# TinyMPC/TinyMPC

Hardware: AMD Instinct MI355X
Metric: QP solves/sec (+ ADMM iters/sec), 64k-batch quadrotor hover (higher is better)
Workload: dtype f64; 1 GPU; quadrotor_hovering (nx=12, nu=4, N=10), 65536 identical instances per GPU, closed-loop MPC steps from a cold start (BASELINE configs[1]); batch_per_gpu=65536, total_batch=65536, parallelism=batch-sharded x1, mpc_steps_per_launch=8, stats_exchange=none (one rank), launcher=plain process

## Files before the change

### tinympc_amd/csrc/admm_kernel.hip.h

```cpp
#pragma once
#include <hip/hip_runtime.h>
#include <stdint.h>

namespace tinympc_amd {

enum : int {
    VEC_CB = 0,
    VEC_CF = 1,
    VEC_QR = 2,
    VEC_SMASK = 3,
    VEC_NIM = 4,
    VEC_SOCFLAG = 5,
    VEC_CONE_BASE = 6,
    VEC_CONE_MU = 7,
    VEC_RHO = 8,
    VEC_LINFLAG = 9,
    VEC_TLINFLAG = 10,
    VEC_COUNT = 16,
};
struct LaneTab {
    int cols, lw;
    constexpr int MB() const { return 0; }
    constexpr int MF1() const { return cols * lw; }
    constexpr int MF2() const { return 2 * cols * lw; }
// ... 361 lines not shown
            DPP_REP(TINYMPC_FUSED_NX, HFWD_COL_A_HI)
            "v_mov_b64 %[xn], %[t]\n\t"
            "v_add_f64 %[gnew], %[tt], -%[vn]\n\t"
            DPP_REP(TINYMPC_FUSED_NU, HFWD_COL_B_LO)
            "s_nop 0\n\t"
            DPP_REP(TINYMPC_FUSED_NU, HFWD_COL_B_HI)
            : [tt] "=&v"(tt), [vm] "=&v"(vm), [vn] "=&v"(vn), [xn] "=&v"(xn), [t] "+&v"(t), [gnew] "=&v"(gnew)
            : [xi] "v"(xi), [g] "v"(g), [lo] "v"(lo), [hi] "v"(hi), FUSED_ROW_OPERANDS);
    }
#endif
}

__device__ __forceinline__ double vmax64(double a, double b) {
    double r;
    asm("v_max_f64 %0, %1, %2" : "=v"(r) : "v"(a), "v"(b));
    return r;
}
__device__ __forceinline__ double vmin64(double a, double b) {
    double r;
    asm("v_min_f64 %0, %1, %2" : "=v"(r) : "v"(a), "v"(b));
    return r;
}
__device__ __forceinline__ double pinned_sub64(double a, double b) {
    double r = a - b;
    asm volatile("" : "+v"(r));
    return r;
}
__device__ __forceinline__ double vclamp64(double lo, double hi, double t) {
    double r;
    asm("v_max_f64 %0, %1, %2\n\tv_min_f64 %0, %3, %0" : "=&v"(r) : "v"(lo), "v"(t), "v"(hi));
    return r;
}

__device__ __forceinline__ double vmax_abs64(double a, double b) {
    double r;
    asm("v_max_f64 %0, %1, |%2|" : "=v"(r) : "v"(a), "v"(b));
    return r;
}
template <bool OPAQUE>
__device__ __forceinline__ double resid_max(double a, double b) {
    if constexpr (OPAQUE) return vmax_abs64(a, b);
    else return fmax(a, fabs(b));
}

#ifndef TINYMPC_PRIM_STORE
#define TINYMPC_PRIM_STORE 1
#endif
#ifndef TINYMPC_REF_LOAD
#define TINYMPC_REF_LOAD 1
#endif
#ifndef TINYMPC_FULL_LINE_STORES
#define TINYMPC_FULL_LINE_STORES 2
#endif
__device__ __forceinline__ double load_ref(const double* p) {
#if TINYMPC_REF_LOAD == 1
    return __builtin_nontemporal_load(p);
#else
    return *p;
#endif
}
__device__ __forceinline__ void store_primal(double* p, double v) {
#if TINYMPC_PRIM_STORE == 1
    __builtin_nontemporal_store(v, p);
#elif TINYMPC_PRIM_STORE == 2
    asm volatile("global_store_dwordx2 %0, %1, off sc1" : : "v"(p), "v"(v) : "memory");
#elif TINYMPC_PRIM_STORE == 3
// ... 792 lines not shown
#pragma unroll
                        for (int s = 0; s < N; ++s) {
                            const double vc0 = soc_lane ? X[s] : 0.0;
                            sC[cw + s * SLOT_D] = vc0 - sC[cw + s * SLOT_D + PL_GC];
                            sC[cw + s * SLOT_D + PL_VC] = vc0;
                        }
                    }
                }
                if constexpr (LS) {
                    if (step > 0) {
#pragma unroll
                        for (int s = 0; s < N; ++s) { if constexpr (LSP) sLV[cl + s * CSL] = lin_lane ? X[s] : 0.0; else VL[s] = lin_lane ? X[s] : 0.0; }
                    } else if (is_state && lin_lane && !resumed) { if constexpr (LSP) sLV[cl] = x0v; else VL[0] = x0v; }
                }
                if constexpr (LT) {
                    if (step > 0) {
#pragma unroll
                        for (int s = 0; s < N; ++s) { if constexpr (LTP) sTV[cl + s * CSL] = tlin_lane ? X[s] : 0.0; else VT[s] = tlin_lane ? X[s] : 0.0; }
                    } else if (is_state && tlin_lane && !resumed) { if constexpr (LTP) sTV[cl] = x0v; else VT[0] = x0v; }
                }
                if constexpr (LPL) __builtin_amdgcn_fence(__ATOMIC_RELEASE, "wavefront");
                const int iter0 = iter_first;
                iter = iter0; solved = 0;
                if (resumed && P.check_termination > 0) checked = 1;
                int countdown = P.check_termination;
                double wr[SOC ? SPR : 1];
                bool gcz[SOC_PASSES];
#pragma unroll
                for (int p = 0; p < SOC_PASSES; ++p) gcz[p] = false;
                if constexpr (SOC) {
#pragma unroll
                    for (int d = 1; d <= SPR && d <= N; ++d) wr[(N - d) % SPR] = sC[cw + (N - d) * SLOT_D];
                }
                for (int it = iter0; it < P.max_iter; ++it) {
                    double lvr[LSP ? SPR : 1], lgr[LSP ? SPR : 1], tvr[LTP ? SPR : 1], tgr[LTP ? SPR : 1];
                    if constexpr (LPL) {
#pragma unroll
                        for (int d = 1; d <= SPR && d <= N; ++d) {
                            if constexpr (LSP) { lvr[(N - d) % SPR] = sLV[cl + (N - d) * CSL]; lgr[(N - d) % SPR] = sLG[cl + (N - d) * CSL]; }
                            if constexpr (LTP) { tvr[(N - d) % SPR] = sTV[cl + (N - d) * CSL]; tgr[(N - d) % SPR] = sTG[cl + (N - d) * CSL]; }
                        }
                    }
                    auto lin_w = [&](const int s_) { if constexpr (LSP) return lvr[s_ % SPR] - lgr[s_ % SPR]; else return VL[LSR ? s_ : 0] - GL[LSR ? s_ : 0]; };
                    auto tlin_w = [&](const int s_) { if constexpr (LTP) return tvr[s_ % SPR] - tgr[s_ % SPR]; else return VT[LTR ? s_ : 0] - GT[LTR ? s_ : 0]; };
                    double qhi;
                    {
                        double t = fma(-rho, VN[N - 1] - G[N - 1], QX[N - 1]);
                        if constexpr (SOC) t = fma(-rho, wr[(N - 1) % SPR], t);
                        if constexpr (LS) t = fma(-rho, lin_w(N - 1), t);
                        if constexpr (LT) t = fma(-rho, tlin_w(N - 1), t);
                        qhi = t;
                        if constexpr (DBG) {
                            double ql = fma(-rho, VN[N - 1] - G[N - 1], qx_last_plain);
                            if constexpr (SOC) ql = fma(-rho, wr[(N - 1) % SPR], ql);
                            if constexpr (LS) ql = fma(-rho, lin_w(N - 1), ql);
                            if constexpr (LT) ql = fma(-rho, tlin_w(N - 1), ql);
                            Qd[N - 1] = is_state ? ql : t;
                            Pd[N - 1] = t;
                        }
                    }
                    double pcur = qhi;
                    if constexpr (HALF) {
                        double tmpv = VN[N - 2] - G[N - 2];
#pragma unroll
                        for (int i = N - 2; i >= 0; --i) {
                            double qlo, res, dnp, tmpn;
                            constexpr int dummy = 0;
// ... 4 lines not shown
                            pcur = res;
                            qhi = qlo;
                        }
                        Dn[0] = fma(pcur, nim, cf);
                    }
#pragma unroll
                    for (int i = N - 2; i >= 0 && !HALF; --i) {
                        if constexpr (SOC) {
                            if (i >= SPD) wr[(i - SPD) % SPR] = sC[cw + (i - SPD) * SLOT_D];
                        }
                        if constexpr (LSP) { if (i >= SPD) { lvr[(i - SPD) % SPR] = sLV[cl + (i - SPD) * CSL]; lgr[(i - SPD) % SPR] = sLG[cl + (i - SPD) * CSL]; } }
                        if constexpr (LTP) { if (i >= SPD) { tvr[(i - SPD) % SPR] = sTV[cl + (i - SPD) * CSL]; tgr[(i - SPD) % SPR] = sTG[cl + (i - SPD) * CSL]; } }
                        if constexpr (SOC || LPL) __builtin_amdgcn_sched_barrier(0);
                        if constexpr (FUSED) {
                            double qlo, res;
                            if constexpr (SOC) fused_backward_step_soc<NX, NU>(qlo, res, VN[i], G[i], QX[i], wr[i % SPR], rho, smask, cb, pcur, qhi, mb, mb + NX);
                            else fused_backward_step<NX, NU>(qlo, res, VN[i], G[i], QX[i], rho, smask, cb, pcur, qhi, mb, mb + NX);
                            pcur = res;
                            Dn[i] = fma(res, nim, cf);
                            if constexpr (DBG) { Qd[i] = qlo; Pd[i] = res; Dd[i + 1] = res; }
                            qhi = qlo;
                            continue;
                        }
                        double qlo = fma(-rho, VN[i] - G[i], QX[i]);
                        if constexpr (SOC) qlo = fma(-rho, wr[i % SPR], qlo);
                        if constexpr (LS) qlo = fma(-rho, lin_w(i), qlo);
                        if constexpr (LT) qlo = fma(-rho, tlin_w(i), qlo);
                        const double res = ring_sum2<MODE, NX, NU>(fma(qlo, smask, cb), pcur, mb, qhi, mb + NX);
                        pcur = res;
                        Dn[i] = fma(res, nim, cf);
                        if constexpr (DBG) { Qd[i] = qlo; Pd[i] = res; Dd[i + 1] = res; }
                        qhi = qlo;
                    }
                    constexpr bool LAZY_RES = N <= 12;
                    constexpr bool TIGHT = FUSED && !HALF && LAZY_RES && !SOC && NX % 4 == 0;
                    double pmax = 0.0, dmax = 0.0;
                    auto slot_update = [&](const int s, const double lo, const double hi, const double gcv, const double glv, const double gtv) {
                        const double xi = X[s];
                        const double t = xi + G[s];
                        const double vn = TIGHT ? vclamp64(lo, hi, t) : vmin64(hi, vmax64(lo, t));
                        if constexpr (!LAZY_RES) {
                            pmax = resid_max<true>(pmax, xi - vn);
                            dmax = resid_max<true>(dmax, VP[s] - vn);
                        }
                        G[s] = t - vn;
                        VN[s] = vn;
                        if constexpr (SOC) {
                            sC[cw + s * SLOT_D] = fma(xi, socmask, gcv);
                        }
                        if constexpr (LSP) sLV[cl + s * CSL] = (lin_lane && (is_state || s >= 1)) ? (xi + glv) : 0.0;
                        if constexpr (LTP) sTV[cl + s * CSL] = (tlin_lane && (is_state || s >= 1)) ? (xi + gtv) : 0.0;
                        if constexpr (LSR || LTR) {
                            auto halfspaces = [&](double z, const double* tabk, const int nk) {
                                for (int k = 0; k < nk; ++k) {
                                    const double a = tabk[k * 16 + j];
                                    const double bk = tabk[KMAX * 16 + k * 16 + j];
                                    const double nn = tabk[2 * KMAX * 16 + k * 16 + j];
                                    const double prod = a * z;
                                    double cs = 0.0, ci = 0.0;
                                    ring1<0, NX>(cs, prod, ones);
                                    ring1<NX, NU>(ci, prod, ones);
                                    const double cv = is_state ? cs : ci;
                                    if (cv > bk) {
#pragma clang fp contract(off)
                                        const double pr = ((cv - bk) / nn) * a;
                                        z = z - pr;
                                    }
                                }
                                return z;
// ... 47 lines not shown
                                if constexpr (!LAZY_RES) {
                                    pmax = resid_max<true>(pmax, xi - vn);
                                    dmax = resid_max<true>(dmax, VP[i] - vn);
                                }
                                G[i] = gnew;
                                VN[i] = vn;
                                lo_c = lo_n; hi_c = hi_n;
                                continue;
                            }
                            fused_forward_step<NX, NU, TIGHT>(tt, vn, t, xn, xi, G[i], lo_c, hi_c, mf1, mf2);
                            X[i + 1] = xn;
                            if constexpr (!LAZY_RES) {
                                pmax = resid_max<true>(pmax, xi - vn);
                                dmax = resid_max<true>(dmax, VP[i] - vn);
                            }
                            if constexpr (TIGHT) {
                                __builtin_amdgcn_sched_barrier(0);
                                if (i > 0) G[i - 1] = pinned_sub64(tt_d, vn_d);
                                tt_d = tt; vn_d = vn;
                            } else G[i] = tt - vn;
                            VN[i] = vn;
                            if constexpr (SOC) sC[cw + i * SLOT_D] = fma(xi, socmask, gr[i % SPR]);
                            lo_c = lo_n; hi_c = hi_n;
                            continue;
                        }
                        const double t = ring_sum<MODE, 0, NX>(Dn[i], X[i], mf1);
                        X[i + 1] = ring_short<MODE, NX, NU>(t, t, mf2);
                        slot_update(i, lo_c, hi_c, gr[SOC ? i % SPR : 0], glr[LSP ? i % SPR : 0], gtr[LTP ? i % SPR : 0]);
                        lo_c = lo_n; hi_c = hi_n;
                    }
                    if constexpr (TIGHT && N >= 2) G[N - 2] = tt_d - vn_d;
                    (void)tt_d; (void)vn_d;
                    slot_update(N - 1, lo_c, hi_c, gr[SOC ? (N - 1) % SPR : 0], glr[LSP ? (N - 1) % SPR : 0], gtr[LTP ? (N - 1) % SPR : 0]);
                    if constexpr (LPL) {
                        __builtin_amdgcn_fence(__ATOMIC_RELEASE, "wavefront");
                        __builtin_amdgcn_wave_barrier();
                        if constexpr (LSP) {
                            if (lin_x_on) project_halfspace_columns<NX, KMAX, 16, 16>(j, grp, N, CSL, 0, 0, sLV, sLG, rLin, 0, P.n_lin);
                            if (lin_u_on) project_halfspace_columns<NU, KMAX, 16, 16>(j, grp, N, CSL, NX, 1, sLV, sLG, rLin, 0, P.n_lin);
                        }
                        if constexpr (LTP) {
                            if (tlin_x_on) project_halfspace_columns<NX, KMAX, 16, 16>(j, grp, N, CSL, 0, 0, sTV, sTG, rTLin, 3 * KMAX * 16, P.n_tlin);
                            if (tlin_u_on) project_halfspace_columns<NU, KMAX, 16, 16>(j, grp, N, CSL, NX, 1, sTV, sTG, rTLin, 3 * KMAX * 16, P.n_tlin);
                        }
                        __builtin_amdgcn_fence(__ATOMIC_RELEASE, "wavefront");
                        __builtin_amdgcn_wave_barrier();
                    }
                    bool conv = false;
                    auto termination = [&]() {
                        if (countdown > 0 && --countdown == 0) {
                            countdown = P.check_termination;
                            checked = 1;
                            constexpr int PS0 = N >= 2 ? 1 : 0, PS1 = N - 1;
                            auto lost = [&](const int s) {
                                return (int)(fabs(X[s] - VN[s]) >= P.tol_pri) | (int)(fabs(VP[s] - VN[s]) * rho >= P.tol_dua);
                            };
                            const bool maybe = ((int)!(rho > 0.0) | (int)!(lost(PS0) | lost(PS1))) != 0;
                            unsigned long long fold = __ballot(maybe);
                            fold &= fold >> 1; fold &= fold >> 2; fold &= fold >> 4;
                            if constexpr (!HALF) fold &= fold >> 8;
                            const bool any_row = (fold & (HALF ? 0x0101010101010101ull : 0x0001000100010001ull)) != 0ull;
                            const bool last_test = (P.max_iter - 1 - it) < P.check_termination;
                            if (last_test || any_row) {
                                if constexpr (LAZY_RES) {
#pragma unroll
                                    for (int s = 0; s < N; ++s) {
                                        pmax = resid_max<false>(pmax, X[s] - VN[s]);
                                        dmax = resid_max<false>(dmax, VP[s] - VN[s]);
                                    }
                                }
                                rp = pmax;
                                rd = dmax * rho;
                                const bool ok = (rp < P.tol_pri) && (rd < P.tol_dua);
                                const unsigned long long bal = __ballot(ok);
                                conv = ((bal >> (grp * RL)) & RMASK) == RMASK;
                            }
                        }
                    };
                    if constexpr (SOC) {
                        __builtin_amdgcn_fence(__ATOMIC_RELEASE, "wavefront");
                        __builtin_amdgcn_wave_barrier();
                        double n0 = sC[item_at[0]], n1 = sC[item_at[0] + 1], n2 = sC[item_at[0] + 2];
#pragma unroll
                        for (int d = 1; d <= SPR && d <= N; ++d) wr[(N - d) % SPR] = sC[cw + (N - d) * SLOT_D];
                        termination();
                        bool any_exact = false;
#pragma unroll
                        for (int p = 0; p < SOC_PASSES; ++p) {
                            if (p > 0 && p >= soc_passes) break;
                            const int at = item_at[p];
                            if (p > 0) { n0 = sC[at]; n1 = sC[at + 1]; n2 = sC[at + 2]; }
                            const double s0 = n0, s1 = n1, s2 = n2;
                            if (soc_all_inside(s0, s1, s2, item_mu[p])) {
                                sC[at + PL_VC] = s0; sC[at + PL_VC + 1] = s1; sC[at + PL_VC + 2] = s2;
                                if (!gcz[p]) {
                                    sC[at + PL_GC] = 0.0; sC[at + PL_GC + 1] = 0.0; sC[at + PL_GC + 2] = 0.0;
                                    gcz[p] = true;
                                }
                            } else {
                                double r0, r1, r2;
                                soc_project3(s0, s1, s2, item_mu[p], item_rmu[p], mu_pow2, r0, r1, r2);
                                const double g0 = s0 - r0, g1 = s1 - r1, g2 = s2 - r2;
                                sC[at + PL_VC] = r0; sC[at + PL_VC + 1] = r1; sC[at + PL_VC + 2] = r2;
                                sC[at + PL_GC] = g0; sC[at + PL_GC + 1] = g1; sC[at + PL_GC + 2] = g2;
                                sC[at] = r0 - g0; sC[at + 1] = r1 - g1; sC[at + 2] = r2 - g2;
                                gcz[p] = false;
                                any_exact = true;
                            }
                        }
                        if (it == iter0 && !proj_lane) {
#pragma unroll
                            for (int s = 0; s < N; ++s) sC[cw + s * SLOT_D + PL_GC] = 0.0;
                        }
                        __builtin_amdgcn_fence(__ATOMIC_RELEASE, "wavefront");
                        __builtin_amdgcn_wave_barrier();
                        if (any_exact) {
#pragma unroll
                            for (int d = 1; d <= SPR && d <= N; ++d) wr[(N - d) % SPR] = sC[cw + (N - d) * SLOT_D];
// ... 41 lines not shown
                            dual_res = grp_max16(dual_res); px_max = grp_max16(px_max); aty_max = grp_max16(aty_max); q_max = grp_max16(q_max);
                            const double pri_norm = fmax(ax_max, z_max);
                            const double dual_norm = fmax(fmax(px_max, aty_max), q_max);
                            const double eps = 1e-10;
                            const double normalized_pri = pri_res / (pri_norm + eps);
                            const double normalized_dual = dual_res / (dual_norm + eps);
                            const double ratio = normalized_pri / (normalized_dual + eps);
                            double new_rho = rho * sqrt(ratio);
                            if (P.aclip) new_rho = fmin(fmax(new_rho, P.arho_min), P.arho_max);
                            const double delta = new_rho - rho;
                            if (is_state) {
#pragma unroll
                                for (int k = 0; k < NU; ++k) mb[NX + k] = -taylor_step(-mb[NX + k], delta, (HA ? atab_i[ATAB_DK + k * 16 + j] : sTab[(16 + j) * AKC + k]));
#pragma unroll
                                for (int k = 0; k < NX; ++k) {
                                    const int e = grp * NX * NX + k + NX * j;
                                    sP[e] = taylor_step(sP[e], delta, (HA ? atab_i[ATAB_DP + k * 16 + j] : sTab[(32 + j) * AKC + k]));
                                }
                            } else if (is_input) {
#pragma unroll
                                for (int k = 0; k < NX; ++k) mf1[k] = -taylor_step(-mf1[k], delta, (HA ? atab_i[ATAB_DK + k * 16 + j] : sTab[(16 + j) * AKC + k]));
                            }
                            if (P.aC1 || P.aC2) {
                                if (j == 0) sDl[grp * ADAPT_LOG + ndl] = delta;
                                if (++ndl == ADAPT_LOG) { flush_c(ndl); ndl = 0; }
                            }
                            rho = new_rho;
                            __builtin_amdgcn_fence(__ATOMIC_RELEASE, "wavefront");
                            __builtin_amdgcn_wave_barrier();
                            QX[N - 1] = qx_last_plain;
                            terminal_term();
                        }
                    }
                    if constexpr (!SOC) termination();
                    if (conv) { solved = 1; break; }
#pragma unroll
                    for (int s = 0; s < N; ++s) VP[s] = VN[s];
                    vp_touched = true;
                }
                acc_iter += (unsigned)(iter - iter0);
                acc_solved += (unsigned)solved;
                if (P.iter_log && j == 0) P.iter_log[(size_t)step * P.batch + b] = solved ? iter : -iter;
                if (P.u0_log && is_input) P.u0_log[((size_t)step * P.batch + b) * NU + (j - NX)] = X[1];
                if constexpr (PE) {
                    double* const elog = late_arg<double>(__builtin_offsetof(SolveArgs, est_log));
                    if (elog && is_state) elog[((size_t)step * P.batch + b) * NX + j] = X[0];
                }
                if (nsteps > 1) {
                    x0v = is_state ? X[1] : 0.0;
                    if constexpr (PM) {
                        if (step + 1 < nsteps) {
                            const size_t cell = true_cell();
                            double xt = true_x0(step, cell);
                            [[maybe_unused]] double est_next = 0.0;
                            if constexpr (PE) est_next = (iter > iter0) ? predicted(X[0], X[1]) : (is_state ? late_arg<double>(__builtin_offsetof(SolveArgs, est_xp))[cell] : 0.0);
                            double ua = X[1];
                            if (iter > iter0) {
                                ua = applied(X[1], step);
                                const double xp = plant_step(xt, ua);
                                xt = is_state ? xp : 0.0;
                                if constexpr (PD) xt = disturbed(xt, step);
                            }
                            if (P.x0_next && is_state) P.x0_next[cell] = xt;
                            if constexpr (PS) { if (iter > iter0) scored(xt, ua, step); }
                            if constexpr (PA) { if (iter > iter0) act_logged(ua, step); }
                            if (P.state_log && is_state) P.state_log[((size_t)step * P.batch + b) * NX + j] = xt;
                            x0v = measured(xt, step + 1);
// ... 161 lines not shown
```

### tinympc_amd/csrc/batch_api.hip

```cpp
#include "batch_impl.hpp"
#include "batch_dispatch.hpp"

#include <cstdarg>
#include <cstdio>
#include <dlfcn.h>
#include <string>
#include <mutex>
#include <cmath>
#include <cstdlib>
#include <cstring>
#include <limits>

namespace tinympc_amd {

__global__ void pack_kpi_kernel(double* __restrict__ kpi, const double* __restrict__ src, int batch, int N,
                                int nz, int rows, int row_off, int cols, int broadcast) {
    const size_t total = (size_t)batch * cols * rows;
    for (size_t e = blockIdx.x * (size_t)blockDim.x + threadIdx.x; e < total; e += (size_t)gridDim.x * blockDim.x) {
        const int r = (int)(e % rows);
        const int i = (int)((e / rows) % cols);
        const size_t b = e / ((size_t)rows * cols);
        const size_t s = broadcast ? ((size_t)i * rows + r) : e;
        kpi[(b * N + i) * nz + row_off + r] = src[s];
    }
// ... 772 lines not shown
    } else if (!strcmp(name, "grid_waves_per_cu")) b->grid_waves_per_cu = (int)value;
    else if (!strcmp(name, "dpp_mode")) b->dpp_mode = (int)value;
    else if (!strcmp(name, "steps_per_launch")) b->steps_per_launch = (int)value;
    else if (!strcmp(name, "force_general")) { b->force_general = value != 0; b->tab_dirty = true; }
    else if (!strcmp(name, "no_jit")) { b->no_jit = value != 0; b->tab_dirty = true; if (!b->no_jit) b->variant_jit_failed = false; }
    else if (!strcmp(name, "no_tile")) { b->no_tile = value != 0; b->tab_dirty = true; }
    else if (!strcmp(name, "prefer_tile")) { b->prefer_tile = value != 0; b->tab_dirty = true; }
    else if (!strcmp(name, "tile_dyn")) b->tile_dyn_opt = (int)value;
    else if (!strcmp(name, "het_ub")) b->het_ub = value != 0;
    else if (!strcmp(name, "tile_w")) b->tile_w = (int)value;
    else if (!strcmp(name, "tile_lm")) b->tile_lm = (int)value;
    else if (!strcmp(name, "tile_r")) b->tile_r = (int)value;
    else if (!strcmp(name, "step_log")) b->step_log = value != 0;
    else if (!strcmp(name, "estimate_log")) b->est.log.on = value != 0;
    else if (!strcmp(name, "actuation_step")) b->anoise.step = value;
    else if (!strcmp(name, "actuation_log")) b->act.log.on = value != 0;
    else if (!strcmp(name, "score_step")) b->score.step = value;
    else if (!strcmp(name, "state_log")) b->plant.log.on = value != 0;
    else if (!strcmp(name, "reset_duals")) b->reset_duals = value != 0;
    else if (!strcmp(name, "store_primal")) { if (value < 0 || value > 2) return fail(b, TINY_ERR_ARG, "store_primal: 0, 1 or 2"); b->store_primal = (int)value; }
    else if (!strcmp(name, "share_ref")) b->share_ref = value != 0;
    else if (!strcmp(name, "half_rows")) b->half_rows = (int)value;
    else if (!strcmp(name, "one_shot_fast")) b->one_shot_fast = value != 0;
    else if (!strcmp(name, "repack_tail")) { if (value < -1 || value > 1) return fail(b, TINY_ERR_ARG, "repack_tail: -1 (by rule), 0 (follow-up stages), 1 (the tile kernel's dynamic form)"); b->repack_tail = (int)value; }
    else if (!strcmp(name, "plan")) { b->plan_opt = value != 0 ? 1 : 0; if (!b->plan_opt) b->plan_tried = true; }
    else if (!strcmp(name, "prefetch")) { if (value < -1 || value > 1) return fail(b, TINY_ERR_ARG, "prefetch: -1 (by rule), 0 (never), 1 (wherever the form exists)"); b->prefetch = (int)value; }
    else if (!strcmp(name, "prefetch_static")) { if (value < -1 || value > 100) return fail(b, TINY_ERR_ARG, "prefetch_static: percent, 0 ... 100, or -1 (by rule: 75 warm, 50 cold)"); b->prefetch_static = (int)value; }
    else if (!strcmp(name, "prefetch_waves")) { if (value < 0) return fail(b, TINY_ERR_ARG, "prefetch_waves >= 0"); b->prefetch_waves = (int)value; }
    else if (!strcmp(name, "launch_order")) { if (value < 0 || value > 2) return fail(b, TINY_ERR_ARG, "launch_order: 0 (ascending), 1 (alternating), 2 (descending)"); b->launch_order = (int)value; }
    else if (!strcmp(name, "step_regroup")) { if (value < -1) return fail(b, TINY_ERR_ARG, "step_regroup: K > 0 (stretches of K MPC steps), 0 (never) or -1 (automatic)"); b->step_regroup = (int)value; b->learn.step_regroup_set(); b->ls_pending = false; }
    else if (!strcmp(name, "step_regroup_streams")) { if (value < 1 || value > 2) return fail(b, TINY_ERR_ARG, "step_regroup_streams: 1 or 2"); b->regroup_streams = (int)value; }
    else if (!strcmp(name, "auto_cold")) b->auto_cold = value != 0;
    else if (!strcmp(name, "uniform_bounds")) b->use_ub = value != 0;
    else if (!strcmp(name, "one_shot")) { if (value < 0 || value > 2) return fail(b, TINY_ERR_ARG, "one_shot: 0, 1 or 2"); b->one_shot = (int)value; }
    else if (!strcmp(name, "repack_after")) { if (value < -1) return fail(b, TINY_ERR_ARG, "repack_after: K > 0, 0 (never) or -1 (automatic)"); b->repack_after = (int)value; b->learn.repack_after_set(); b->hist_pending = false; if (value < 0 && b->plan_opt) { b->plan_tried = false; b->plan_shipped = false; } }
    else if (!strcmp(name, "repack_waves_per_cu")) b->repack_waves_per_cu = (int)std::max(1L, value);
    else if (!strcmp(name, "repack_growth")) { b->repack_growth = (int)value; b->learn.repack_growth_set(); }
    else if (!strcmp(name, "repack_sort")) { if (value < -1 || value > 1) return fail(b, TINY_ERR_ARG, "repack_sort: 1, 0 or -1 (automatic)"); b->repack_sort = (int)value; }
    else if (!strcmp(name, "repack_dynamic")) b->repack_dynamic = value != 0;
    else if (!strcmp(name, "traj_step")) b->traj_step = value;
    else if (!strcmp(name, "measurement_step")) b->meas.step = value;
    else if (!strcmp(name, "disturbance_step")) b->dist.step = value;
    else if (!strcmp(name, "timing")) {
        HIP_TRY(b, hipStreamSynchronize(b->stream));
        while ((long)b->ev_start.size() < value) {
            hipEvent_t s, e;
            HIP_TRY(b, hipEventCreate(&s));
            HIP_TRY(b, hipEventCreate(&e));
            b->ev_start.push_back(s); b->ev_stop.push_back(e);
        }
        b->timing_n = 0;
        b->timing_left = (int)value;
    } else return fail(b, TINY_ERR_ARG, "unknown option %s", name);
    return TINY_OK;
}

int tiny_batch_set_stream(TinyBatch* b, void* hip_stream) {
    if (!b) return TINY_ERR_NULL;
    HIP_TRY(b, hipSetDevice(b->device));
    HIP_TRY(b, hipStreamSynchronize(b->stream));
    if (b->own_stream && b->stream) hipStreamDestroy(b->stream);
    b->stream = (hipStream_t)hip_stream;
    b->own_stream = false;
    return TINY_OK;
}

// ... 102 lines not shown
    if (!strcmp(name, "n_input_linear")) return b->nil;
    if (!strcmp(name, "n_tv_state_linear")) return b->ntsl;
    if (!strcmp(name, "n_tv_input_linear")) return b->ntil;
    if (!strcmp(name, "instance_linear")) return (b->ilin.on[0] ? 1 : 0) | (b->ilin.on[1] ? 2 : 0);
    if (!strcmp(name, "last_instance_linear")) return b->ilin.last;
    if (!strcmp(name, "n_state_cones")) return (long)b->Acx.size();
    if (!strcmp(name, "n_input_cones")) return (long)b->Acu.size();
    if (!strcmp(name, "instance_cones")) return b->icone.on ? 1 : 0;
    if (!strcmp(name, "last_instance_cones")) return b->icone.last ? 1 : 0;
    if (!strcmp(name, "disturbance")) return b->dist.seq ? b->dist.steps : 0;
    if (!strcmp(name, "disturbance_step")) return b->dist.step;
    if (!strcmp(name, "disturbance_generated")) return (b->dist.seq && b->dist.generated) ? 1 : 0;
    if (!strcmp(name, "measurement_noise_generated")) return (b->meas.seq && b->meas.generated) ? 1 : 0;
    if (!strcmp(name, "last_disturbance")) return b->dist.last ? 1 : 0;
    if (!strcmp(name, "measurement_noise")) return b->meas.seq ? b->meas.steps : 0;
    if (!strcmp(name, "measurement_step")) return b->meas.step;
    if (!strcmp(name, "last_measurement_noise")) return b->meas.last ? 1 : 0;
    if (!strcmp(name, "plant")) return b->plant.kind;
    if (!strcmp(name, "last_plant")) return b->plant.last ? 1 : 0;
    if (!strcmp(name, "state_log")) return b->plant.log.on ? 1 : 0;
    if (!strcmp(name, "estimator")) return b->est.kind;
    if (!strcmp(name, "last_estimator")) return b->est.last ? 1 : 0;
    if (!strcmp(name, "estimate_log")) return b->est.log.on ? 1 : 0;
    if (!strcmp(name, "score")) return b->score.kind;
    if (!strcmp(name, "score_step")) return b->score.step;
    if (!strcmp(name, "last_score")) return b->score.last ? 1 : 0;
    if (!strcmp(name, "actuator")) return b->act.kind;
    if (!strcmp(name, "actuator_lag")) return (b->act.kind && b->act.lag) ? 1 : 0;
    if (!strcmp(name, "actuation_noise")) return b->anoise.seq ? b->anoise.steps : 0;
    if (!strcmp(name, "actuation_noise_generated")) return (b->anoise.seq && b->anoise.generated) ? 1 : 0;
    if (!strcmp(name, "actuation_step")) return b->anoise.step;
    if (!strcmp(name, "last_actuator")) return b->act.last ? 1 : 0;
    if (!strcmp(name, "actuation_log")) return b->act.log.on ? 1 : 0;
    if (!strcmp(name, "last_uniform_bounds")) return b->last_ub ? 1 : 0;
    if (!strcmp(name, "auto_split_measured_permille")) return (b->learn.auto_plain_rate > 0.0 && b->learn.auto_split_rate > 0.0) ? (long)(1000.0 * b->learn.auto_split_rate / b->learn.auto_plain_rate + 0.5) : 0;
    if (!strcmp(name, "repack_after")) return b->repack_after;
    if (!strcmp(name, "repack_sorted_stages")) return b->last_sorted_stages;
    if (!strcmp(name, "step_regroup")) return b->step_regroup;
    if (!strcmp(name, "step_regroup_stretches")) return b->last_regroup_stretches;
    if (!strcmp(name, "step_regroup_verdict") || !strcmp(name, "lockstep_permille")) {
        if (b->ls_pending && hipEventSynchronize(b->ls_ev) == hipSuccess) read_lockstep_estimate(b);
        return name[0] == 's' ? (long)b->learn.regroup_verdict : (long)(b->learn.lockstep_ratio * 1000.0 + 0.5);
    }
    return fail(b, TINY_ERR_ARG, "unknown option %s", name);
}

int tiny_batch_get_plan(TinyBatch* b, TinyBatchPlan* out) {
    if (!b || !out) return TINY_ERR_NULL;
    HIP_TRY(b, hipSetDevice(b->device));
    if (b->hist_pending && hipEventSynchronize(b->hist_ev) == hipSuccess) learn_from_probe(b, b->set.max_iter, true);
    if (b->ls_pending && hipEventSynchronize(b->ls_ev) == hipSuccess) read_lockstep_estimate(b);
    memset(out, 0, sizeof(*out));
    out->magic = TINY_PLAN_MAGIC; out->version = TINY_PLAN_VERSION; out->bytes = (int)sizeof(TinyBatchPlan);
    out->nx = b->nx; out->nu = b->nu; out->N = b->N; out->batch = b->batch;
    out->max_iter = b->set.max_iter; out->check_termination = b->set.check_termination;
    b->learn.to_plan(out, b->repack_growth);
    return TINY_OK;
}

int tiny_batch_set_plan(TinyBatch* b, const TinyBatchPlan* in) {
    if (!b || !in) return TINY_ERR_NULL;
    if (in->magic != TINY_PLAN_MAGIC || in->version != TINY_PLAN_VERSION || in->bytes != (int)sizeof(TinyBatchPlan))
        return fail(b, TINY_ERR_ARG, "not a TinyBatchPlan of this library version");
    if (in->nx != b->nx || in->nu != b->nu || in->N != b->N)
        return fail(b, TINY_ERR_DIM, "the plan was made for (nx,nu,N)=(%d,%d,%d), this batch is (%d,%d,%d)", in->nx, in->nu, in->N, b->nx, b->nu, b->N);
    if (!LaunchLearner::plan_in_range(in)) return fail(b, TINY_ERR_ARG, "TinyBatchPlan: field out of range");
// ... 96 lines not shown
```

### tinympc_amd/csrc/batch_dispatch.hip

```cpp
#define TINYMPC_GENERAL_KERNEL_IMPL
#include "batch_impl.hpp"
#include "batch_dispatch.hpp"

#include <algorithm>
#include <cstdarg>
#include <cstdio>
#include <cstring>
#include <limits>
#include <string>

namespace tinympc_amd {

#include "_gen/registry.inc"
const int g_nkernels = (int)(sizeof(g_kernels) / sizeof(g_kernels[0]));
const KernelEntry* const* const g_kernel_list = g_kernels;

static const int g_ntiles = (int)(sizeof(g_tiles) / sizeof(g_tiles[0]));
const TileEntry* find_tile(int nx, int nu, int N) {
    for (int i = 0; i < g_ntiles; ++i)
        if (g_tiles[i]->nx == nx && g_tiles[i]->nu == nu && g_tiles[i]->N == N) return g_tiles[i];
    return nullptr;
}
static int variant_tile_r(const TinyBatch* b) {
    int r = b->tile ? b->tile->R : 1;
// ... 224 lines not shown
static int bind_tile_args(TinyBatch* b, const TileLaunch& T, SolveArgs& a) {
    a = {};
    a.tab = b->d_ttab;
    if (int rc = bind_common_args(b, a)) return rc;
    if (T.lin) { if (int rc = bind_halfspace_slacks(b, T.lin, a)) return rc; }
    a.het_tabs = b->hetero ? b->d_het_tabs : nullptr;
    a.cold = b->one_shot ? 1 : 0;
    if (b->one_shot && (T.lm & TILE_LM_VPG)) {
        if (!b->d_vz_scratch) {
            const size_t bytes = (size_t)b->batch * b->N * (b->nx + b->nu) * sizeof(double) + (size_t)b->N * (b->nx + b->nu) * sizeof(double) + 1024;
            HIP_TRY(b, hipMalloc(&b->d_vz_scratch, bytes));
            HIP_TRY(b, hipMemsetAsync(b->d_vz_scratch, 0, bytes, b->stream));
        }
        a.vz_stream = b->d_vz_scratch;
    }
    return TINY_OK;
}

static int enqueue_tile(TinyBatch* b, const TileLaunch& T, SolveArgs a, int batch) {
    a.batch = batch;
    if (T.dyn) {
        if (!b->d_work_counter) HIP_TRY(b, hipMalloc(reinterpret_cast<void**>(&b->d_work_counter), sizeof(int)));
        HIP_TRY(b, hipMemsetAsync(b->d_work_counter, 0, sizeof(int), b->stream));
        a.work_counter = b->d_work_counter;
    }
    if (T.jit_fn) {
        void* params[] = {&a};
        HIP_TRY(b, hipModuleLaunchKernel(T.jit_fn, (unsigned)T.grid, 1, 1, 64, 1, 1, 0, b->stream, params, nullptr));
    } else {
        hipLaunchKernelGGL(T.k, dim3(T.grid), dim3(64), 0, b->stream, a);
        HIP_TRY(b, hipGetLastError());
    }
    b->last_tile_dyn = T.dyn;
    b->last_ub = T.jit_fn ? T.ub : (T.te && ((T.te->kub && T.k == T.te->kub) || (T.te->kubdyn && T.k == T.te->kubdyn)));
    b->last_tile_form = T.te ? (T.te->W * 1000000 + T.te->R * 1000 + T.te->lm) : -1;
    return TINY_OK;
}

static int run_tile_launch(TinyBatch* b, const TileLaunch& T, SolveArgs a) {
    if (first_launch_of(b, T.key())) { if (int rc = enqueue_tile(b, T, a, 0)) return rc; }
    if (b->tail_index) {
        a.index = b->tail_index; a.count = b->tail_count; a.iter_base = b->tail_iter_base;
        return enqueue_tile(b, T, a, b->batch);
    }
    bool timed = false;
    if (int rc = timing_begin(b, &timed)) return rc;
    if (int rc = enqueue_tile(b, T, a, b->batch)) return rc;
    if (int rc = timing_end(b, timed)) return rc;
    b->status_valid = true;
    if (b->d_traj) b->traj_step += a.steps;
    return TINY_OK;
}

static int prepare_tile_launch(TinyBatch* b, TileLaunch& T, SolveArgs& a, bool& done) {
    if (int rc = upload_tile_tables(b)) return rc;
    std::string why;
    switch (decide_tile_launch(b, T, why)) {
    case TILE_GO:
        return bind_tile_args(b, T, a);
    case TILE_NO_ENTRY:
        return fail(b, TINY_ERR_UNSUPPORTED, "no compiled-in tile kernel form for (%d,%d,%d)", b->nx, b->nu, b->N);
    case TILE_HET_LAYOUT:
        return fail(b, TINY_ERR_UNSUPPORTED, "per-instance tables were built as %d x %d, the tile kernel form about to run reads 32 x %d", b->het_tab_cols, b->het_tab_lw, 16 * T.W);
    case TILE_EXT_REFUSED:
        b->tile_soc_failed = true;
        return fail(b, TINY_ERR_UNSUPPORTED, "the tile kernel's form for per-instance data / reference windows / reset_duals / one_shot could not be instantiated for (%d,%d,%d): %s",
// ... 66 lines not shown
    if (*p) return TINY_OK;
    const size_t kpi_bytes = (size_t)b->batch * b->N * (b->nx + b->nu) * sizeof(double);
    HIP_TRY(b, hipMalloc(p, kpi_bytes));
    HIP_TRY(b, hipMemsetAsync(*p, 0, kpi_bytes, b->stream));
    return TINY_OK;
}

static __global__ void general_prestep_kernel(double* __restrict__ ref, double* __restrict__ dual, const double* __restrict__ traj,
                                              const int* __restrict__ offsets, int points, int k, int batch, int N, int nx, int nz, int reset) {
    const size_t total = (size_t)batch * N * nz;
    for (size_t e = blockIdx.x * (size_t)blockDim.x + threadIdx.x; e < total; e += (size_t)gridDim.x * blockDim.x) {
        const int j = (int)(e % nz), i = (int)((e / nz) % N);
        const size_t bb = e / ((size_t)nz * N);
        if (traj && j < nx) {
            int kk = k + (offsets ? offsets[bb] : 0) + i;
            kk = kk < points ? kk : points - 1;
            ref[e] = traj[(size_t)kk * nx + j];
        }
        if (reset) dual[e] = 0.0;
    }
}
static __global__ void general_step_log_kernel(const int4* __restrict__ status, const double* __restrict__ prim, int* __restrict__ iter_log,
                                               double* __restrict__ u0_log, int batch, int N, int nx, int nu) {
    for (int bb = blockIdx.x * blockDim.x + threadIdx.x; bb < batch; bb += gridDim.x * blockDim.x) {
        const int4 st = status[bb];
        iter_log[bb] = st.y ? st.x : -st.x;
        for (int a = 0; a < nu; ++a) u0_log[(size_t)bb * nu + a] = prim[(size_t)bb * N * (nx + nu) + nx + a];
    }
}

int launch_general(TinyBatch* b, int phase) {
    if (b->nx + b->nu > 32) return fail(b, TINY_ERR_UNSUPPORTED, "nx + nu = %d > 32", b->nx + b->nu);
    const int gsteps = (phase == 0 && b->steps_per_launch > 1) ? b->steps_per_launch : 1;
    if (phase == 0) b->last_ub = false;
    if (int rc = ensure_instance_data(b)) return rc;
    if (phase == 0) note_instance_data_read(b);
    if (phase == 0 && gsteps > 1 && b->step_log) { if (int rc = ensure_step_logs(b, gsteps)) return rc; }
    CoverageLoop stages;
    if (phase == 0) { if (int rc = coverage_begin(b, gsteps, stages)) return rc; }
    double** need[] = {&b->d_dbg_qr, &b->d_dbg_pd, &b->d_lslack, &b->d_ldual, &b->d_tlslack, &b->d_tldual};
    const int lf = lin_families(b), sf = soc_families(b);
    const bool want[] = {true, true, (lf & 1) != 0, (lf & 1) != 0, (lf & 2) != 0, (lf & 2) != 0};
    for (int i = 0; i < 6; ++i)
        if (want[i]) { if (int rc = ensure_kpi(b, need[i])) return rc; }
    if (b->tab_dirty || b->h_gtab.empty() || phase > 0) {
        build_general_tables(b);
        if (int rc = upload_growing(b, &b->d_gtab, &b->gtab_doubles, b->h_gtab)) return rc;
    }
    GeneralArgs a = b->gargs;
    a.gtab = b->d_gtab; a.x0 = b->d_x0; a.ref = b->d_ref; a.prim = b->d_prim; a.slack = b->d_slack; a.dual = b->d_dual;
    a.slack_prev = b->d_slack_prev; a.cslack = b->d_cslack; a.cdual = b->d_cdual; a.lslack = b->d_lslack; a.ldual = b->d_ldual;
    a.tlslack = b->d_tlslack; a.tldual = b->d_tldual; a.qr = b->d_dbg_qr; a.pd = b->d_dbg_pd;
    a.status = b->d_status; a.resid = b->d_resid; a.accum = b->d_accum; a.x0_next = ((b->advance_x0 || gsteps > 1) && !stages.own_plant) ? b->d_x0 : nullptr;
    a.rho = b->cache.rho; a.tol_pri = b->set.abs_pri_tol; a.tol_dua = b->set.abs_dua_tol;
    a.batch = b->batch; a.max_iter = b->set.max_iter; a.check_termination = b->set.check_termination;
    a.nx = b->nx; a.nu = b->nu; a.N = b->N;
    a.soc_s = (sf >> 1) & 1; a.soc_i = sf & 1;
    a.n_sc = b->set.en_state_soc ? (int)b->Acx.size() : 0; a.n_ic = b->set.en_input_soc ? (int)b->Acu.size() : 0;
    a.lin_s = b->set.en_state_linear; a.lin_i = b->set.en_input_linear;
    a.tlin_s = b->set.en_tv_state_linear; a.tlin_i = b->set.en_tv_input_linear;
    a.nsl = b->nsl; a.nil = b->nil; a.ntsl = b->ntsl; a.ntil = b->ntil;
    a.het_tabs = b->hetero ? b->d_het_tabs : nullptr;
    a.het_cols = b->het_tab_cols; a.het_lw = b->het_tab_lw; a.het_stride = b->hetero ? LaneTab{b->het_tab_cols, b->het_tab_lw}.het_doubles() : 0;
    a.inst_bounds = b->ibox.on ? b->ibox.built : nullptr; a.ib_lw = box_lanes(b->nx, b->nu);
    a.inst_lin = inst_lin_active(b) ? b->ilin.built : nullptr;
    a.il_stride = b->ilin.stride; a.il_lw = box_lanes(b->nx, b->nu); a.il_km = b->ilin.km; a.il_lv = b->ilin.lv;
    a.inst_cones = inst_cones_active(b) ? b->icone.built : nullptr; a.ic_lw = box_lanes(b->nx, b->nu);
// ... 63 lines not shown
constexpr int PF_AUTO_MIN_TILES = 3;
struct OneRowLaunch {
    SolveArgs a = {};
    SolveKernel k = nullptr;
    hipFunction_t jit_fn = nullptr;
    JitKey jk;
    int steps = 1, ipw = 4, grid = 0;
    bool soc = false;
    SolveKernel kpf = nullptr;
    int pf_grid = 0, pf_mask = 0, pf_tiles = 0;
    size_t pf_lds = 0;
    bool use_pf = false;
    bool split_ok = false, auto_split = false, growth_probe = false, auto_probe = false;
    bool tail_tile = false;
    TileLaunch tail;
    int cap = 0;
};

static int bind_one_row_args(TinyBatch* b, const PathDecision& D, const bool zero_state, OneRowLaunch& L) {
    b->h_gtab.clear();
    if (int rc = upload_tables(b)) return rc;
    const bool soc = L.soc = soc_active(b);
    SolveArgs& a = L.a;
    a.pf_shards = 1; a.pf_static = 1;
    a.tab = b->d_tab;
    if (int rc = bind_common_args(b, a)) return rc;
    L.steps = a.steps;
    a.het_tabs = b->hetero ? b->d_het_tabs : nullptr;
    if (b->hetero && (b->het_tab_cols != 16 || b->het_tab_lw != 16))
        return fail(b, TINY_ERR_UNSUPPORTED, "per-instance tables were built as %d x %d, the one-row kernel reads 16 x 16", b->het_tab_cols, b->het_tab_lw);
    a.cold = (b->one_shot || (zero_state && b->auto_cold)) ? 1 : 0;
    a.ref_shared = (b->share_ref && b->xref_shared && b->uref_shared) ? 1 : 0;
    if (b->store_primal != 1 && !b->one_shot && !soc && !D.lin && !b->debug) a.store_mask = (a.store_mask & ~1) | (b->store_primal == 2 ? 32 : 0);
    a.dbg_qr = b->debug ? b->d_dbg_qr : nullptr;
    a.dbg_pd = b->debug ? b->d_dbg_pd : nullptr;
    if (D.lin) {
        if (int rc = bind_halfspace_slacks(b, D.lin, a)) return rc;
        if (D.pl) a.inst_lin = b->ilin.built;
    }
    if (b->adaptive) {
        if (b->one_shot || b->repack_after > 0) return fail(b, TINY_ERR_UNSUPPORTED, "%s", PATH_REFUSAL_MESSAGE[REFUSE_ADAPTIVE_HALFSPACES]);
        if (int rc = ensure_adaptive(b)) return rc;
        a.arho = b->d_arho; a.aK = b->d_aK; a.aP = b->d_aP; a.aC1 = b->d_aC1; a.aC2 = b->d_aC2;
        a.atab = b->hetero ? b->d_atabs : b->d_atab;
        a.arho_min = b->adaptive_min; a.arho_max = b->adaptive_max; a.aclip = b->adaptive_clip ? 1 : 0;
        b->astate_fresh = false;
    }
    if (D.pb) a.inst_bounds = b->ibox.built;
    if (D.pc) a.inst_cones = b->icone.built;
    if (int rc = bind_closed_loop_args(b, D, a)) return rc;
    return TINY_OK;
}
static VariantFacts variant_facts(const TinyBatch* b, const PathDecision& D, const OneRowLaunch& L) {
    VariantFacts f;
    f.lin = D.lin; f.pl = D.pl != 0; f.pb = D.pb != 0; f.pc = D.pc != 0; f.pd = D.pd != 0; f.pp = D.pp != 0; f.pm = D.pm != 0; f.pe = D.pe != 0; f.ps = D.ps != 0; f.pa = D.pa != 0;
    f.soc = L.soc; f.debug = b->debug; f.dpp_mode = b->dpp_mode; f.hetero = b->hetero; f.adaptive = b->adaptive;
    f.lin_kmax = D.lin ? lin_kmax(b) : 0;
    f.il_km = D.pl ? b->ilin.km : 0;
    f.uniform_ub = b->bounds_uniform && b->use_ub;
    f.het_ub = b->het_ub; f.half_rows = b->half_rows != 0; f.no_jit = b->no_jit; f.variant_jit_failed = b->variant_jit_failed;
    f.prefetch_on = b->prefetch != 0; f.single_step = L.steps == 1; f.no_ref_window = !L.a.traj; f.default_grid = b->grid_waves_per_cu == 0;
    return f;
}
static void size_prefetch_launch(TinyBatch* b, SolveKernel c, OneRowLaunch& L) {
    const SolveArgs& a = L.a;
    const bool own = !a.ref_shared;
// ... 27 lines not shown
        else jit_fn = jit_solve_kernel(jk, &why);
        if (!jit_fn && c.fallback.slot != SLOT_NONE) { jk.ub = 0; ub_form = false; k = slot_kernel(b->kernel, c.fallback); b->het_ub = false; }
        if (!jit_fn && !k) {
            if (b->kernel) {
                const bool general_can = !jk.adapt;
                if (general_can && !b->variant_jit_failed) {
                    b->variant_jit_failed = true;
                    b->tab_dirty = true; b->redispatch = true;
                    done = true;
                    return launch_solve(b);
                }
                return fail(b, TINY_ERR_UNSUPPORTED, "this combination of cone / debug outputs / half-spaces / per-instance data / launch form needs hipRTC: %s", why.c_str());
            }
            if (b->adaptive) return fail(b, TINY_ERR_UNSUPPORTED, "adaptive rho kernel for (nx,nu,N)=(%d,%d,%d) could not be instantiated: %s", b->nx, b->nu, b->N, why.c_str());
            b->jit_failed = true;
            b->tab_dirty = true; b->redispatch = true;
            done = true;
            return launch_solve(b);
        }
    }
    b->last_ub = ub_form;
    return TINY_OK;
}
static int build_one_row_launch(TinyBatch* b, const PathDecision& D, const bool zero_state, OneRowLaunch& L, bool& done) {
    if (int rc = bind_one_row_args(b, D, zero_state, L)) return rc;
    const VariantChoice c = choose_one_row_variant(variant_facts(b, D, L), entry_slots(b->kernel));
    L.jk = c.key;
    L.jk.nx = b->nx; L.jk.nu = b->nu; L.jk.N = b->N;
    L.ipw = c.ipw;
    b->last_half = c.ipw == 8;
    L.grid = launch_waves(b, b->batch, c.ipw);
    b->last_prefetch = false;
    if (c.prefetch.slot != SLOT_NONE) size_prefetch_launch(b, slot_kernel(b->kernel, c.prefetch), L);
    return resolve_one_row_variant(b, c, L, done);
}

void learn_from_probe(TinyBatch* b, const int max_iter, const bool auto_split) {
    if (auto_split && b->hist_pending && hipEventQuery(b->hist_ev) == hipSuccess) {
        b->hist_pending = false;
        float ms = 0.0f;
        const bool have_reading = hipEventElapsedTime(&ms, b->auto_ev0, b->auto_ev1) == hipSuccess;
        b->learn.probe_arrived(have_reading, ms, b->h_hist, max_iter, split_model(b));
    }
}

static bool one_row_layout_tile_ok(const TinyBatch* b, const OneRowLaunch& L) {
    return b->tile && !b->tile_is_jit && b->tile->W <= 1 && !b->no_tile && !L.soc && !L.jk.lin && !L.jk.het && !L.jk.adapt && !L.jk.dbg && !L.jk.pb &&
           !b->d_traj && !b->reset_duals && b->store_primal == 1;
}
struct DynamicTileFormGuard {
    TinyBatch* const b;
    const int dyn, lm, r;
    explicit DynamicTileFormGuard(TinyBatch* b_, const int* index = nullptr, const int* count = nullptr, int iter_base = 0)
        : b(b_), dyn(b_->tile_dyn_opt), lm(b_->tile_lm), r(b_->tile_r) {
        b->tile_dyn_opt = 1; b->tile_lm = -1; b->tile_r = 0;
        b->tail_index = index; b->tail_count = count; b->tail_iter_base = iter_base;
    }
    ~DynamicTileFormGuard() { b->tile_dyn_opt = dyn; b->tile_lm = lm; b->tile_r = r; b->tail_index = nullptr; b->tail_count = nullptr; b->tail_iter_base = 0; }
};

static int try_tile_alternative(TinyBatch* b, const OneRowLaunch& L, bool& done) {
    if (!(L.auto_split && one_row_layout_tile_ok(b, L) && b->tile_dyn_opt < 0 && !b->prefer_tile && b->repack_after < 0)) return TINY_OK;
    const bool probe_tile = b->learn.tile_probe_wanted(b->repack_growth, b->hist_pending);
    if (b->learn.tile_verdict != 1 && !probe_tile) return TINY_OK;
    if (b->learn.tile_solve_counted()) return TINY_OK;
    DynamicTileFormGuard guard(b);
    TileLaunch T;
// ... 289 lines not shown
```

### tinympc_amd/csrc/batch_impl.hpp

```cpp
#pragma once
#include <hip/hip_runtime.h>

#include <vector>

#include "../../include/tinympc_amd.h"
#include "kernel_entry.hpp"
#include "general_kernel.hip.h"
#include "jit.hpp"
#include "riccati_kernel.hip.h"
#include "sensitivity_kernel.hip.h"
#include "tile_kernel.hip.h"
#include "cache.hpp"
#include "launch_learner.hpp"
#include "closed_loop.hpp"

namespace tinympc_amd {

struct Settings {
    double abs_pri_tol = 1e-3, abs_dua_tol = 1e-3;
    int max_iter = 1000, check_termination = 1;
    int en_state_bound = 1, en_input_bound = 1, en_state_soc = 0, en_input_soc = 0;
    int en_state_linear = 0, en_input_linear = 0, en_tv_state_linear = 0, en_tv_input_linear = 0;
};

// ... 63 lines not shown
    void* d_kpi_slab = nullptr;
    int4* d_status = nullptr;
    uint2* d_accum = nullptr;
    double *d_lslack = nullptr, *d_ldual = nullptr, *d_tlslack = nullptr, *d_tldual = nullptr, *d_gtab = nullptr;
    size_t gtab_doubles = 0, general_lds_limit = 0, phase_lds_limit = 0;
    std::vector<double> h_gtab;
    tinympc_amd::GeneralArgs gargs;
    bool force_general = false;
    int* d_iter_log = nullptr;
    double* d_u0_log = nullptr;
    int log_steps = 0;
    size_t stage_doubles = 0;
    std::vector<double> h_tab;
    bool tab_dirty = true;
    unsigned tab_gen = 1, ttab_gen = 0;
    int last_path = -1;
    bool advance_x0 = false, debug = false;
    int grid_waves_per_cu = 0, dpp_mode = 2, steps_per_launch = 1;
    bool step_log = false, reset_duals = false;
    int repack_after = -1;
    enum { HIST_BINS = 1024 };
    unsigned *d_hist = nullptr, *h_hist = nullptr;
    hipEvent_t hist_ev = nullptr;
    bool hist_pending = false;
    hipEvent_t auto_ev0 = nullptr, auto_ev1 = nullptr;
    bool repack_dynamic = false;
    int repack_waves_per_cu = 8, repack_growth = 0;
    int repack_sort = -1;
    int last_sorted_stages = 0;
    int *d_repack_index = nullptr, *d_repack_count = nullptr;
    bool use_ub = true;
    bool bounds_uniform = false;
    bool last_ub = false;
    InstanceBox ibox; InstanceHalfspaces ilin; InstanceCones icone;
    Disturbance dist; PlantStep plant; MeasurementNoise meas; Estimator est; Score score; Actuator act; StepSequence anoise; ModelBlock model;
    bool xref_shared = true, uref_shared = true;
    bool share_ref = true;
    int half_rows = -1;
    bool last_half = false;
    int launch_order = 1;
    bool order_flip = false;
    int prefetch = -1, prefetch_waves = 0;
    int prefetch_static = -1;
    unsigned* d_pf_counter = nullptr;
    unsigned pf_base[8] = {0, 0, 0, 0, 0, 0, 0, 0};
    bool last_prefetch = false;
    int plan_opt = 1;
    int het_tab_cols = 0, het_tab_lw = 0;
    bool one_shot_fast = true;
    double* d_vz_scratch = nullptr;
    int repack_tail = -1;
    const int* tail_index = nullptr;
    const int* tail_count = nullptr;
    int tail_iter_base = 0;
    bool last_tail_tile = false;
    const void* loaded_kernels[6] = {nullptr, nullptr, nullptr, nullptr, nullptr, nullptr};
    bool helpers_loaded = false;
    bool plan_tried = false, plan_shipped = false;
    int last_pf_grid = 0;
    size_t last_pf_lds = 0;
    const void* pf_occ_kernel = nullptr;
    size_t pf_occ_lds = 0;
    int pf_occ = 0;
    int step_regroup = -1;
    bool status_valid = false;
    int* d_perm = nullptr;
// ... 46 lines not shown
```

Baseline: 2.884 billion QP solves/s.

## Add uniform inner ADMM loop that skips LDS sync when no row can converge

Adds an inner loop to the TIGHT ADMM iteration path. When check_termination is 1, it runs a cheap ballot probe on two slots. If no row of the wavefront can have converged, it copies VN into VP and runs the next iteration immediately, skipping the LDS fences, wave barriers and the full residual reduction. A new uniform_loop option, on by default, sets bit 256 of store_mask to enable it, and the host records when the variant applies. The cost is a more complex control flow with a possible rise in register pressure, and the probe must stay exact so termination behaviour is unchanged.

```diff
diff --git a/tinympc_amd/csrc/admm_kernel.hip.h b/tinympc_amd/csrc/admm_kernel.hip.h
--- a/tinympc_amd/csrc/admm_kernel.hip.h
+++ b/tinympc_amd/csrc/admm_kernel.hip.h
@@ -417,6 +417,9 @@
     return r;
 }
 
+template <bool B>
+struct flag_arg { static constexpr bool value = B; };
+
 __device__ __forceinline__ double vmax_abs64(double a, double b) {
     double r;
     asm("v_max_f64 %0, %1, |%2|" : "=v"(r) : "v"(a), "v"(b));
@@ -1275,7 +1278,57 @@
 #pragma unroll
                     for (int d = 1; d <= SPR && d <= N; ++d) wr[(N - d) % SPR] = sC[cw + (N - d) * SLOT_D];
                 }
+                [[maybe_unused]] const int uni_end = ((P.store_mask & 256) != 0 && P.check_termination == 1) ? P.max_iter : 0;
                 for (int it = iter0; it < P.max_iter; ++it) {
+                    [[maybe_unused]] int uni_ran = 0;
+                    constexpr bool LAZY_RES = N <= 12;
+                    constexpr bool TIGHT = FUSED && !HALF && LAZY_RES && !SOC && NX % 4 == 0;
+                    constexpr bool UNI = TIGHT && !DBG && !ADAPT && !(PD || PP || PM || PE || PS || PA);
+                    double pmax = 0.0, dmax = 0.0;
+                    bool conv;
+                    auto termination = [&](auto probe_only) {
+                        constexpr bool PROBE = decltype(probe_only)::value;
+                        if (PROBE || (countdown > 0 && --countdown == 0)) {
+                            if constexpr (!PROBE) {
+                                countdown = P.check_termination;
+                                checked = 1;
+                            }
+                            bool any_row = true;
+                            if (PROBE || !UNI || !(it + 1 < uni_end)) {
+                                constexpr int PS0 = N >= 2 ? 1 : 0, PS1 = N - 1;
+                                auto lost = [&](const int s) {
+                                    return (int)(fabs(X[s] - VN[s]) >= P.tol_pri) | (int)(fabs(VP[s] - VN[s]) * rho >= P.tol_dua);
+                                };
+                                const bool maybe = ((int)!(rho > 0.0) | (int)!(lost(PS0) | lost(PS1))) != 0;
+                                unsigned long long fold = __ballot(maybe);
+                                if constexpr (UNI) {
+                                    fold = (~fold - 0x0001000100010001ull) & fold & 0x8000800080008000ull;
+                                } else {
+                                    fold &= fold >> 1; fold &= fold >> 2; fold &= fold >> 4;
+                                    if constexpr (!HALF) fold &= fold >> 8;
+                                }
+                                any_row = (fold & (HALF ? 0x0101010101010101ull : UNI ? ~0ull : 0x0001000100010001ull)) != 0ull;
+                            }
+                            if constexpr (PROBE) return any_row;
+                            const bool last_test = (P.max_iter - 1 - it) < P.check_termination;
+                            if (last_test || any_row) {
+                                if constexpr (LAZY_RES) {
+#pragma unroll
+                                    for (int s = 0; s < N; ++s) {
+                                        pmax = resid_max<false>(pmax, X[s] - VN[s]);
+                                        dmax = resid_max<false>(dmax, VP[s] - VN[s]);
+                                    }
+                                }
+                                rp = pmax;
+                                rd = dmax * rho;
+                                const bool ok = (rp < P.tol_pri) && (rd < P.tol_dua);
+                                const unsigned long long bal = __ballot(ok);
+                                conv = ((bal >> (grp * RL)) & RMASK) == RMASK;
+                            }
+                        }
+                        if constexpr (PROBE) return false;
+                    };
+                    for (;;) {
                     double lvr[LSP ? SPR : 1], lgr[LSP ? SPR : 1], tvr[LTP ? SPR : 1], tgr[LTP ? SPR : 1];
                     if constexpr (LPL) {
 #pragma unroll
@@ -1346,9 +1399,6 @@
                         if constexpr (DBG) { Qd[i] = qlo; Pd[i] = res; Dd[i + 1] = res; }
                         qhi = qlo;
                     }
-                    constexpr bool LAZY_RES = N <= 12;
-                    constexpr bool TIGHT = FUSED && !HALF && LAZY_RES && !SOC && NX % 4 == 0;
-                    double pmax = 0.0, dmax = 0.0;
                     auto slot_update = [&](const int s, const double lo, const double hi, const double gcv, const double glv, const double gtv) {
                         const double xi = X[s];
                         const double t = xi + G[s];
@@ -1462,6 +1512,17 @@
                     if constexpr (TIGHT && N >= 2) G[N - 2] = tt_d - vn_d;
                     (void)tt_d; (void)vn_d;
                     slot_update(N - 1, lo_c, hi_c, gr[SOC ? (N - 1) % SPR : 0], glr[LSP ? (N - 1) % SPR : 0], gtr[LTP ? (N - 1) % SPR : 0]);
+                    if constexpr (!UNI) break;
+                    else {
+                        if (__builtin_expect(!(it + 1 < uni_end && !termination(flag_arg<true>())), 1)) break;
+#pragma unroll
+                        for (int s = 0; s < N; ++s) VP[s] = VN[s];
+                        ++it; ++uni_ran;
+                    }
+                    }
+                    if constexpr (UNI) {
+                        if (uni_ran > 0) { iter += uni_ran; checked = 1; vp_touched = true; }
+                    }
                     if constexpr (LPL) {
                         __builtin_amdgcn_fence(__ATOMIC_RELEASE, "wavefront");
                         __builtin_amdgcn_wave_barrier();
@@ -1476,44 +1537,14 @@
                         __builtin_amdgcn_fence(__ATOMIC_RELEASE, "wavefront");
                         __builtin_amdgcn_wave_barrier();
                     }
-                    bool conv = false;
-                    auto termination = [&]() {
-                        if (countdown > 0 && --countdown == 0) {
-                            countdown = P.check_termination;
-                            checked = 1;
-                            constexpr int PS0 = N >= 2 ? 1 : 0, PS1 = N - 1;
-                            auto lost = [&](const int s) {
-                                return (int)(fabs(X[s] - VN[s]) >= P.tol_pri) | (int)(fabs(VP[s] - VN[s]) * rho >= P.tol_dua);
-                            };
-                            const bool maybe = ((int)!(rho > 0.0) | (int)!(lost(PS0) | lost(PS1))) != 0;
-                            unsigned long long fold = __ballot(maybe);
-                            fold &= fold >> 1; fold &= fold >> 2; fold &= fold >> 4;
-                            if constexpr (!HALF) fold &= fold >> 8;
-                            const bool any_row = (fold & (HALF ? 0x0101010101010101ull : 0x0001000100010001ull)) != 0ull;
-                            const bool last_test = (P.max_iter - 1 - it) < P.check_termination;
-                            if (last_test || any_row) {
-                                if constexpr (LAZY_RES) {
-#pragma unroll
-                                    for (int s = 0; s < N; ++s) {
-                                        pmax = resid_max<false>(pmax, X[s] - VN[s]);
-                                        dmax = resid_max<false>(dmax, VP[s] - VN[s]);
-                                    }
-                                }
-                                rp = pmax;
-                                rd = dmax * rho;
-                                const bool ok = (rp < P.tol_pri) && (rd < P.tol_dua);
-                                const unsigned long long bal = __ballot(ok);
-                                conv = ((bal >> (grp * RL)) & RMASK) == RMASK;
-                            }
-                        }
-                    };
+                    conv = false;
                     if constexpr (SOC) {
                         __builtin_amdgcn_fence(__ATOMIC_RELEASE, "wavefront");
                         __builtin_amdgcn_wave_barrier();
                         double n0 = sC[item_at[0]], n1 = sC[item_at[0] + 1], n2 = sC[item_at[0] + 2];
 #pragma unroll
                         for (int d = 1; d <= SPR && d <= N; ++d) wr[(N - d) % SPR] = sC[cw + (N - d) * SLOT_D];
-                        termination();
+                        termination(flag_arg<false>());
                         bool any_exact = false;
 #pragma unroll
                         for (int p = 0; p < SOC_PASSES; ++p) {
@@ -1621,7 +1652,7 @@
                             terminal_term();
                         }
                     }
-                    if constexpr (!SOC) termination();
+                    if constexpr (!SOC) termination(flag_arg<false>());
                     if (conv) { solved = 1; break; }
 #pragma unroll
                     for (int s = 0; s < N; ++s) VP[s] = VN[s];
diff --git a/tinympc_amd/csrc/batch_api.hip b/tinympc_amd/csrc/batch_api.hip
--- a/tinympc_amd/csrc/batch_api.hip
+++ b/tinympc_amd/csrc/batch_api.hip
@@ -828,6 +828,7 @@
     else if (!strcmp(name, "step_regroup_streams")) { if (value < 1 || value > 2) return fail(b, TINY_ERR_ARG, "step_regroup_streams: 1 or 2"); b->regroup_streams = (int)value; }
     else if (!strcmp(name, "auto_cold")) b->auto_cold = value != 0;
     else if (!strcmp(name, "uniform_bounds")) b->use_ub = value != 0;
+    else if (!strcmp(name, "uniform_loop")) b->uniform_loop = value != 0;
     else if (!strcmp(name, "one_shot")) { if (value < 0 || value > 2) return fail(b, TINY_ERR_ARG, "one_shot: 0, 1 or 2"); b->one_shot = (int)value; }
     else if (!strcmp(name, "repack_after")) { if (value < -1) return fail(b, TINY_ERR_ARG, "repack_after: K > 0, 0 (never) or -1 (automatic)"); b->repack_after = (int)value; b->learn.repack_after_set(); b->hist_pending = false; if (value < 0 && b->plan_opt) { b->plan_tried = false; b->plan_shipped = false; } }
     else if (!strcmp(name, "repack_waves_per_cu")) b->repack_waves_per_cu = (int)std::max(1L, value);
@@ -996,6 +997,8 @@
     if (!strcmp(name, "actuation_step")) return b->anoise.step;
     if (!strcmp(name, "last_actuator")) return b->act.last ? 1 : 0;
     if (!strcmp(name, "actuation_log")) return b->act.log.on ? 1 : 0;
+    if (!strcmp(name, "uniform_loop")) return b->uniform_loop ? 1 : 0;
+    if (!strcmp(name, "last_uniform_loop")) return b->last_uniform_loop ? 1 : 0;
     if (!strcmp(name, "last_uniform_bounds")) return b->last_ub ? 1 : 0;
     if (!strcmp(name, "auto_split_measured_permille")) return (b->learn.auto_plain_rate > 0.0 && b->learn.auto_split_rate > 0.0) ? (long)(1000.0 * b->learn.auto_split_rate / b->learn.auto_plain_rate + 0.5) : 0;
     if (!strcmp(name, "repack_after")) return b->repack_after;
diff --git a/tinympc_amd/csrc/batch_dispatch.hip b/tinympc_amd/csrc/batch_dispatch.hip
--- a/tinympc_amd/csrc/batch_dispatch.hip
+++ b/tinympc_amd/csrc/batch_dispatch.hip
@@ -280,6 +280,7 @@
         HIP_TRY(b, hipGetLastError());
     }
     b->last_tile_dyn = T.dyn;
+    b->last_uniform_loop = false;
     b->last_ub = T.jit_fn ? T.ub : (T.te && ((T.te->kub && T.k == T.te->kub) || (T.te->kubdyn && T.k == T.te->kubdyn)));
     b->last_tile_form = T.te ? (T.te->W * 1000000 + T.te->R * 1000 + T.te->lm) : -1;
     return TINY_OK;
@@ -412,7 +413,7 @@
 int launch_general(TinyBatch* b, int phase) {
     if (b->nx + b->nu > 32) return fail(b, TINY_ERR_UNSUPPORTED, "nx + nu = %d > 32", b->nx + b->nu);
     const int gsteps = (phase == 0 && b->steps_per_launch > 1) ? b->steps_per_launch : 1;
-    if (phase == 0) b->last_ub = false;
+    if (phase == 0) { b->last_ub = false; b->last_uniform_loop = false; }
     if (int rc = ensure_instance_data(b)) return rc;
     if (phase == 0) note_instance_data_read(b);
     if (phase == 0 && gsteps > 1 && b->step_log) { if (int rc = ensure_step_logs(b, gsteps)) return rc; }
@@ -542,6 +543,7 @@
     a.cold = (b->one_shot || (zero_state && b->auto_cold)) ? 1 : 0;
     a.ref_shared = (b->share_ref && b->xref_shared && b->uref_shared) ? 1 : 0;
     if (b->store_primal != 1 && !b->one_shot && !soc && !D.lin && !b->debug) a.store_mask = (a.store_mask & ~1) | (b->store_primal == 2 ? 32 : 0);
+    if (b->uniform_loop) a.store_mask |= 256;
     a.dbg_qr = b->debug ? b->d_dbg_qr : nullptr;
     a.dbg_pd = b->debug ? b->d_dbg_pd : nullptr;
     if (D.lin) {
@@ -635,7 +637,12 @@
     L.grid = launch_waves(b, b->batch, c.ipw);
     b->last_prefetch = false;
     if (c.prefetch.slot != SLOT_NONE) size_prefetch_launch(b, slot_kernel(b->kernel, c.prefetch), L);
-    return resolve_one_row_variant(b, c, L, done);
+    if (int rc = resolve_one_row_variant(b, c, L, done)) return rc;
+    const JitKey& k = L.jk;
+    if (!done)
+        b->last_uniform_loop = (L.a.store_mask & 256) && L.a.check_termination == 1 && k.mode == 2 && !k.soc && !k.dbg && !k.lin && !k.adapt &&
+                               c.ipw != 8 && b->N <= 12 && b->nx % 4 == 0 && !k.pd && !k.pp && !k.pm && !k.pe && !k.ps && !k.pa;
+    return TINY_OK;
 }
 
 void learn_from_probe(TinyBatch* b, const int max_iter, const bool auto_split) {
diff --git a/tinympc_amd/csrc/batch_impl.hpp b/tinympc_amd/csrc/batch_impl.hpp
--- a/tinympc_amd/csrc/batch_impl.hpp
+++ b/tinympc_amd/csrc/batch_impl.hpp
@@ -119,6 +119,8 @@
     bool use_ub = true;
     bool bounds_uniform = false;
     bool last_ub = false;
+    bool uniform_loop = true;
+    bool last_uniform_loop = false;
     InstanceBox ibox; InstanceHalfspaces ilin; InstanceCones icone;
     Disturbance dist; PlantStep plant; MeasurementNoise meas; Estimator est; Score score; Actuator act; StepSequence anoise; ModelBlock model;
     bool xref_shared = true, uref_shared = true;
```

Result: slower. 2.825 billion QP solves/s (-2.1%).
